# acids-ircam/RAVE

Hardware: NVIDIA H100
Metric: audio-seconds/s (v2 train step fwd+bwd, 48 kHz) (higher is better)
Workload: dtype bf16

## Files before the change

### include/rave_b200.h

```cpp
#ifndef RAVE_B200_H
#define RAVE_B200_H

#include <stddef.h>
#include <stdint.h>

#ifdef __cplusplus
extern "C" {
#endif

#define RAVE_ACT_NONE 0
#define RAVE_ACT_LEAKY 1
#define RAVE_ACT_SNAKE 2

#define RAVE_PREC_FP32 0
#define RAVE_PREC_BF16 1
#define RAVE_PREC_TF32 2

int rave_b200_version(void);
const char *rave_b200_last_error(void);
unsigned long long rave_b200_launch_count(void);

int rave_pqmf_analysis_fwd(const float *x, const float *taps, float *y, int B, int T, int Lout,
                           int ntaps, int pad_l, int flip_sign, void *stream);
int rave_pqmf_synthesis_fwd(const float *x, const float *w, float *out, int B, int L, int K,
// ... 18 lines not shown
int rave_conv1d_wgrad_f32(const float *P, const float *Q, float *dw, int B, int Ca, int Lp, int Cc,
                          int Lq, int K, int stride, int dil, int pad_l, long os_a, long os_c,
                          int act_p, int act_q, float slope, const float *alpha, void *workspace,
                          void *stream);

int rave_weight_norm_fwd(const float *v, const float *g, float *w, float *norm_out, int C0, int R,
                         void *stream);
int rave_weight_norm_bwd(const float *dw, const float *v, const float *g, const float *norm,
                         float *dv, float *dg, int C0, int R, void *stream);

int rave_act_fwd(const float *x, float *y, int B, int C, int L, int act, float slope,
                 const float *alpha, void *stream);
int rave_act_bwd(const float *dy, const float *x, float *dx, float *dalpha, int B, int C, int L,
                 int act, float slope, const float *alpha, void *stream);
int rave_am_tanh_fwd(const float *x, float *y, int B, int C, int L, void *stream);
int rave_am_tanh_bwd(const float *dy, const float *x, float *dx, int B, int C, int L, void *stream);
int rave_reparam_fwd(const float *z, const float *eps, float *zs, float *kl_sum, int B, int C, int L, void *stream);
int rave_mmd_fwd(const float *z, const float *prior, float *means, float *mmd, int B, int D, int L, void *stream);
int rave_mmd_bwd(const float *z, const float *prior, const float *g, float *dz, int B, int D, int L, void *stream);
int rave_sphere_norm_fwd(const float *z, float *out, float *norm, int B, int C, int L, void *stream);
int  rave_latent_moments(const float *z, int B, int C, int L, int D, double *state, double *work, void *stream);
long rave_latent_moments_workspace_bytes(int B, int L, int D);
int rave_sphere_norm_bwd(const float *g, const float *out, const float *norm, float *dz, int B, int C, int L,
                         void *stream);

int rave_conv1d_tc_supported(int Cin, int Cout, int K, int stride, int dil);
int rave_dilated_unit_tc_supported(int C, int L);
int rave_dilated_unit_tc_fwd(const void *xa_bf16, const void *w3t_bf16, const void *w1t_bf16, void *a1_out,
                             float *out_f32, void *out_act, int B, int C, int L, int pitch, int dil, int pad_l,
                             float slope_in, float slope_mid, int act_out, float slope_out, void *stream);
int rave_conv1d_tc_plan(int B, int Cin, int Cout, int Lout, int K);
int rave_conv1d_tc_pp_stages(int B, int Cin, int Cout, int Lout, int K, int fm, int res_bf16);
int rave_conv1d_tc_pp_fwd_stages(int B, int Cin, int Cout, int Lout, int K);
int rave_conv1d_tc_fwd(const void *xa_bf16, const void *wt_bf16, const float *bias, const float *res,
                       const void *res_bf16, const void *dact_src_bf16, const void *res_act_bf16, float res_slope,
                       float *out_f32, void *out_act_bf16,
                       int B, int Cin, int Lin, int in_pitch, int Cout, int Lout,
                       int K, int stride, int dil, int pad_l, int act, float slope, int out_rows,
                       int out_row_stride, int out_row_offset, const float *fm_d, int fm_bh, void *stream);
int rave_conv1d_tc_fwd_x3(const void *xa_bf16, const void *wt_bf16, const float *bias, const float *res,
                          const void *res_act, float res_slope, float *out_f32, void *out_act, int B, int Cin, int Lin,
                          int in_pitch, int Cout, int Lout, int K, int stride, int dil, int pad_l, int act, float slope,
                          int out_rows, int out_row_stride, int out_row_offset, int act_cs, void *stream);
int rave_conv1d_tc_wgrad_splits(int B, int Cm, int Lp, int Cn, int K);
int rave_conv1d_tc_wgrad_plan(int B, int Cm, int Lp, int Cn, int K);
int rave_time_stack_cl(const float *x, void *out_bf16, int B, int C, int T, int F, int Fp, int Cp, int kt, int pt,
                       void *stream);
int rave_time_stack_cl_bwd(const void *g_bf16, float *gx, int B, int C, int T, int F, int Fp, int Cp, int kt, int pt,
                           void *stream);
int rave_time_stack_nhwc(const float *x, void *out_bf16, int B, int C, int T, int F, long sb, long st, int Fp, int Cp, int kt,
                         int pt, void *stream);
int rave_time_stack_nhwc_bwd(const void *g_bf16, float *gx, int B, int C, int T, int F, int Fp, int Cp, int kt, int pt,
                             void *stream);
int rave_time_stack_nhwc_dil(const float *x, void *out_bf16, int B, int C, int T, int F, long sb, long st, int Fp, int Cp,
                             int kt, int pt, int dil, void *stream);
int rave_time_stack_nhwc_dil_bwd(const void *g_bf16, float *gx, int B, int C, int T, int F, int Fp, int Cp, int kt, int pt,
                                 int dil, void *stream);
int rave_l1_stats_f32(const float *t, const float *v, float *stats, long n, void *stream);
int rave_l1_grad_f32(const float *t, const float *v, const float *d, float *gt, float *gv, long n, void *stream);
int rave_leaky_fm_fwd(const float *x, float *a, float *stats, long H, float slope, void *stream);
int rave_leaky_fm_bwd(const float *a, const float *g, const float *d, float *gx, long H, float slope, void *stream);
int rave_leaky_fm_stack_fwd(const float *x, float *a, float *stats, void *xs_bf16, long Rh, int T, int F, int C, int Fp,
                            float slope, void *stream);
int rave_leaky_fm_stack_bwd(const float *a, const void *gxs_bf16, const float *ga, const float *d, float *gx, long Rh, int T,
                            int F, int C, int Fp, float slope, void *stream);
int rave_leaky_fm_stack_dil_fwd(const float *x, float *a, float *stats, void *xs_bf16, long Rh, int T, int F, int C, int Fp,
// ... 136 lines not shown
```

### rave_b200/_lib.py

```python
import ctypes
import os
from ctypes import c_float, c_int, c_long, c_longlong, c_size_t, c_ulonglong, c_void_p, c_char_p

_HERE = os.path.dirname(os.path.abspath(__file__))
LIB_PATH = os.path.join(_HERE, "csrc", "librave_b200.so")

_P, _I, _F, _L = c_void_p, c_int, c_float, c_long

SIGNATURES = {
    "rave_b200_version": (c_int, []),
    "rave_b200_last_error": (c_char_p, []),
    "rave_b200_launch_count": (c_ulonglong, []),
    "rave_pqmf_analysis_fwd": (c_int, [_P, _P, _P, _I, _I, _I, _I, _I, _I, _P]),
    "rave_pqmf_synthesis_fwd": (c_int, [_P, _P, _P, _I, _I, _I, _I, _F, _I, _P]),
    "rave_pqmf_analysis_fast": (c_int, [_P, _P, _P, _P, _I, _I, _I, _I, _I, _P]),
    "rave_pqmf_synthesis_fast": (c_int, [_P, _P, _P, _P, _I, _I, _I, _F, _I, _P]),
    "rave_conv1d_gather_f32": (c_int, [_P, _P, _P, _P, _P, _I, _I, _I, _I, _I, _I, _I, _I, _I, _L, _L,
                                       _I, _F, _P, _I, _F, _P, _P, _P]),
    "rave_conv1d_scatter_f32": (c_int, [_P, _P, _P, _P, _P, _I, _I, _I, _I, _I, _I, _I, _I, _I, _L, _L,
                                        _I, _F, _P, _I, _F, _P, _P, _P]),
    "rave_conv1d_wgrad_workspace_bytes": (c_size_t, [_I, _I, _I, _I, _I]),
    "rave_conv1d_wgrad_f32": (c_int, [_P, _P, _P, _I, _I, _I, _I, _I, _I, _I, _I, _I, _L, _L, _I, _I,
                                      _F, _P, _P, _P]),
    "rave_weight_norm_fwd": (c_int, [_P, _P, _P, _P, _I, _I, _P]),
    "rave_weight_norm_bwd": (c_int, [_P, _P, _P, _P, _P, _P, _I, _I, _P]),
    "rave_act_fwd": (c_int, [_P, _P, _I, _I, _I, _I, _F, _P, _P]),
    "rave_act_bwd": (c_int, [_P, _P, _P, _P, _I, _I, _I, _I, _F, _P, _P]),
    "rave_am_tanh_fwd": (c_int, [_P, _P, _I, _I, _I, _P]),
    "rave_am_tanh_bwd": (c_int, [_P, _P, _P, _I, _I, _I, _P]),
    "rave_reparam_fwd": (c_int, [_P, _P, _P, _P, _I, _I, _I, _P]),
    "rave_mmd_fwd": (c_int, [_P, _P, _P, _P, _I, _I, _I, _P]),
    "rave_mmd_bwd": (c_int, [_P, _P, _P, _P, _I, _I, _I, _P]),
    "rave_sphere_norm_fwd": (c_int, [_P, _P, _P, _I, _I, _I, _P]),
    "rave_sphere_norm_bwd": (c_int, [_P, _P, _P, _P, _I, _I, _I, _P]),
    "rave_latent_moments": (c_int, [_P, _I, _I, _I, _I, _P, _P, _P]),
    "rave_latent_moments_workspace_bytes": (c_long, [_I, _I, _I]),
    "rave_conv1d_tc_supported": (c_int, [_I, _I, _I, _I, _I]),
    "rave_dilated_unit_tc_supported": (c_int, [_I, _I]),
    "rave_dilated_unit_tc_fwd": (c_int, [_P, _P, _P, _P, _P, _P, _I, _I, _I, _I, _I, _I, _F, _F, _I, _F, _P]),
    "rave_conv1d_tc_plan": (c_int, [_I, _I, _I, _I, _I]),
    "rave_conv1d_tc_pp_stages": (c_int, [_I, _I, _I, _I, _I, _I, _I]),
    "rave_conv1d_tc_pp_fwd_stages": (c_int, [_I, _I, _I, _I, _I]),
    "rave_conv1d_tc_fwd": (c_int, [_P, _P, _P, _P, _P, _P, _P, _F, _P, _P, _I, _I, _I, _I, _I, _I, _I, _I, _I, _I, _I,
                                   _F, _I, _I, _I, _P, _I, _P]),
    "rave_conv1d_tc_fwd_x3": (c_int, [_P, _P, _P, _P, _P, _F, _P, _P, _I, _I, _I, _I, _I, _I, _I, _I, _I, _I, _I, _F, _I,
                                      _I, _I, _I, _P]),
    "rave_weight_prep_tc_multi_x3": (c_int, [_I, _P, _P]),
    "rave_ncl_to_cl_x3": (c_int, [_P, _P, _I, _I, _I, _P]),
    "rave_conv1d_tc_wgrad": (c_int, [_P, _P, _P, _P, _I, _I, _I, _I, _I, _I, _I, _I, _I, _I, _I, _P]),
    "rave_tapmajor_to_weight_f32": (c_int, [_P, _P, _I, _I, _I, _I, _I, _P]),
    "rave_conv1d_tc_wgrad_splits": (c_int, [_I, _I, _I, _I, _I]),
    "rave_conv1d_tc_wgrad_plan": (c_int, [_I, _I, _I, _I, _I]),
    "rave_time_stack_cl": (c_int, [_P, _P, _I, _I, _I, _I, _I, _I, _I, _I, _P]),
    "rave_time_stack_cl_bwd": (c_int, [_P, _P, _I, _I, _I, _I, _I, _I, _I, _I, _P]),
    "rave_time_stack_nhwc": (c_int, [_P, _P, _I, _I, _I, _I, ctypes.c_long, ctypes.c_long, _I, _I, _I, _I, _P]),
    "rave_time_stack_nhwc_bwd": (c_int, [_P, _P, _I, _I, _I, _I, _I, _I, _I, _I, _P]),
    "rave_time_stack_nhwc_dil": (c_int, [_P, _P, _I, _I, _I, _I, ctypes.c_long, ctypes.c_long, _I, _I, _I, _I, _I, _P]),
    "rave_time_stack_nhwc_dil_bwd": (c_int, [_P, _P, _I, _I, _I, _I, _I, _I, _I, _I, _I, _P]),
    "rave_l1_stats_f32": (c_int, [_P, _P, _P, ctypes.c_long, _P]),
    "rave_leaky_fm_fwd": (c_int, [_P, _P, _P, ctypes.c_long, ctypes.c_float, _P]),
    "rave_leaky_fm_bwd": (c_int, [_P, _P, _P, _P, ctypes.c_long, ctypes.c_float, _P]),
    "rave_leaky_fm_stack_fwd": (c_int, [_P, _P, _P, _P, ctypes.c_long, _I, _I, _I, _I, ctypes.c_float, _P]),
    "rave_leaky_fm_stack_bwd": (c_int, [_P, _P, _P, _P, _P, ctypes.c_long, _I, _I, _I, _I, ctypes.c_float, _P]),
    "rave_leaky_fm_stack_dil_fwd": (c_int, [_P, _P, _P, _P, ctypes.c_long, _I, _I, _I, _I, _I, ctypes.c_float, _P]),
    "rave_leaky_fm_stack_dil_bwd": (c_int, [_P, _P, _P, _P, _P, ctypes.c_long, _I, _I, _I, _I, _I, ctypes.c_float, _P]),
    "rave_l1_grad_f32": (c_int, [_P, _P, _P, _P, _P, ctypes.c_long, _P]),
    "rave_snake_cl_fwd": (c_int, [_P, _P, _P, ctypes.c_long, _I, _P]),
    "rave_snake_cl_bwd": (c_int, [_P, _P, _P, _P, _P, _P, ctypes.c_long, _I, _P]),
    "rave_adain_cl_stats": (c_int, [_P, _I, _I, _I, _I, _P, _P, _P, _P, _P, _P, _P, _P, _I, _P, _P, _P]),
    "rave_adain_snake_cl_fwd": (c_int, [_P, _P, _P, _P, _P, _I, _I, _I, _I, _P]),
    "rave_weight_prep_tc": (c_int, [_P, _P, _P, _P, _P, _I, _P, _P, _I, _I, _I, _I, _I, _I, _P]),
    "rave_weight_norm_bwd_tapmajor": (c_int, [_P, _P, _P, _P, _P, _P, _I, _I, _I, _I, _I, _I, _P]),
    "rave_conv1d_c1_fwd": (c_int, [_P, _P, _P, _P, _P, _I, _I, _I, _I, _I, _I, _I, _I, _I, _I, _F, _P]),
    "rave_conv1d_c1_wgrad_splits": (c_int, [_I, _I]),
    "rave_conv1d_c1_wgrad": (c_int, [_P, _P, _P, _I, _I, _I, _I, _I, _I, _I, _I, _I, _I, _P]),
# ... 127 lines not shown
```

### rave_b200/csrc/conv_tc.cu

```cuda
#include <string.h>

#include <type_traits>

#include "common.cuh"
#include "tc_common.cuh"

namespace rave {
namespace tc {

constexpr int BLOCK_M = 128;
constexpr int NUM_THREADS = 288;
constexpr int SMEM_MAX = 227 * 1024;

struct TcParams {
  int B, Cin, Lin, Cout, Lout, K, stride, dil, pad_l;
  int BL, BB;
  int n_lt, n_bg, n_nt;
  int num_kb;
  int act;
  float slope;
  const float *bias;
  const float *res;
  const __nv_bfloat16 *res_bf16;
  const __nv_bfloat16 *dact_src;
// ... 227 lines not shown

struct Ring {
  uint64_t *full, *empty;
  int stages;
  int stage;
  uint32_t phase;
  __device__ __forceinline__ void advance() {
    if (++stage == stages) { stage = 0; phase ^= 1; }
  }
};

template <int BLOCK_N, int BLOCK_K, bool X3>
__device__ __forceinline__ void produce_kblock(uint8_t *smem, Ring &r, const CUtensorMap *tmap_a,
                                               const CUtensorMap *tmap_b, const TcParams &p, const TileCoord &t,
                                               TapOrigin o, int k, int kb) {
  using L = SmemLayout<BLOCK_N, BLOCK_K, X3>;
  mbar_wait(&r.empty[r.stage], r.phase ^ 1);
  uint8_t *sa = smem + r.stage * L::STAGE_BYTES;
  uint8_t *sb = sa + L::A_BYTES;
  uint64_t *bar = &r.full[r.stage];
  if (elect_one()) {
    mbar_arrive_expect_tx(bar, L::A_BYTES + L::B_BYTES);
    tma_load_4d(sa, tmap_a, bar, kb * BLOCK_K, o.ph, t.l0 + o.j, t.b0);
    tma_load_2d(sb, tmap_b, bar, kb * BLOCK_K, k * p.Cout + t.n0);
    if (X3) {
      tma_load_4d(sa + L::A_PART, tmap_a, bar, p.Cin + kb * BLOCK_K, o.ph, t.l0 + o.j, t.b0);
      tma_load_2d(sb + L::B_PART, tmap_b, bar, kb * BLOCK_K, (p.K + k) * p.Cout + t.n0);
    }
  }
  __syncwarp();
  r.advance();
}

template <int BLOCK_N, int BLOCK_K, bool X3>
__device__ __forceinline__ void mma_kblock(float (*d)[BLOCK_N / 2], uint32_t sa, int kb) {
  using L = SmemLayout<BLOCK_N, BLOCK_K, X3>;
  constexpr int SWZ = BLOCK_K * 2;
  constexpr uint64_t A_HALF = (64 * SWZ) >> 4;
  const uint64_t adesc = make_kmajor_desc(sa, SWZ);
  const uint64_t bdesc = make_kmajor_desc(sa + L::A_BYTES, SWZ);
  wgmma_fence();
#pragma unroll
  for (int kk = 0; kk < BLOCK_K / 16; ++kk) {
#pragma unroll
    for (int h = 0; h < 2; ++h)
      Wgmma<BLOCK_N, 0, 0>::mma(d[h], adesc + h * A_HALF + 2 * kk, bdesc + 2 * kk, (kb > 0 || kk > 0) ? 1u : 0u);
  }
  if (X3) {
    const uint64_t adesc_lo = make_kmajor_desc(sa + L::A_PART, SWZ);
    const uint64_t bdesc_lo = make_kmajor_desc(sa + L::A_BYTES + L::B_PART, SWZ);
#pragma unroll
    for (int kk = 0; kk < BLOCK_K / 16; ++kk) {
#pragma unroll
      for (int h = 0; h < 2; ++h) {
        Wgmma<BLOCK_N, 0, 0>::mma(d[h], adesc_lo + h * A_HALF + 2 * kk, bdesc + 2 * kk, 1u);
        Wgmma<BLOCK_N, 0, 0>::mma(d[h], adesc + h * A_HALF + 2 * kk, bdesc_lo + 2 * kk, 1u);
      }
    }
  }
  wgmma_commit();
}

template <int BLOCK_N, int BLOCK_K, bool X3>
__device__ __forceinline__ int mma_mainloop(float (*d)[BLOCK_N / 2], uint32_t smem_base, Ring &r, int kblocks,
                                            int lane) {
  using L = SmemLayout<BLOCK_N, BLOCK_K, X3>;
  int prev = 0;
  for (int kb = 0; kb < kblocks; ++kb) {
    mbar_wait(&r.full[r.stage], r.phase);
    mma_kblock<BLOCK_N, BLOCK_K, X3>(d, smem_base + r.stage * L::STAGE_BYTES, kb);
    wgmma_wait<1>();
    if (kb > 0) {
      __syncwarp();
      if (lane == 0) mbar_arrive(&r.empty[prev]);
    }
    prev = r.stage;
    r.advance();
  }
  return prev;
}

template <int BLOCK_N>
__device__ __forceinline__ void mma_drain(float (*d)[BLOCK_N / 2], const Ring &r, int prev, int lane) {
  wgmma_wait<0>();
  wgmma_fence_regs<BLOCK_N / 2>(d[0]);
  wgmma_fence_regs<BLOCK_N / 2>(d[1]);
  __syncwarp();
  if (lane == 0) mbar_arrive(&r.empty[prev]);
}

template <int BLOCK_N, int BLOCK_K, bool X3>
__global__ void __launch_bounds__(NUM_THREADS, 1)
conv_tc_kernel(const __grid_constant__ CUtensorMap tmap_a, const __grid_constant__ CUtensorMap tmap_b,
               const __grid_constant__ CUtensorMap tmap_o, const TcParams p) {
  using L = SmemLayout<BLOCK_N, BLOCK_K, X3>;
  const int STAGES = p.stages;
  static_assert(BLOCK_N % 16 == 0 && BLOCK_N >= 16 && BLOCK_N <= 128, "invalid wgmma N");

  extern __shared__ uint8_t smem_raw[];
  uint8_t *smem = reinterpret_cast<uint8_t *>((reinterpret_cast<uintptr_t>(smem_raw) + 1023) & ~uintptr_t(1023));
  uint64_t *full_bar = reinterpret_cast<uint64_t *>(smem + p.bar_off);
  uint64_t *empty_bar = full_bar + STAGES;
  uint64_t *tfull_bar = empty_bar + STAGES;
  uint64_t *tempty_bar = tfull_bar + 2;
  uint8_t *stg = (!X3 && p.stg) ? smem + p.stg_off : nullptr;

  const int warp = threadIdx.x >> 5;
  const int lane = threadIdx.x & 31;
  const int num_tiles = p.n_lt * p.n_bg * p.n_nt;
  const int kblocks = p.K * p.num_kb;

  if (threadIdx.x == 0) {
    tma_prefetch_desc(&tmap_a);
    tma_prefetch_desc(&tmap_b);
    if (stg) tma_prefetch_desc(&tmap_o);
    for (int s = 0; s < STAGES; ++s) {
      mbar_init(&full_bar[s], 1);
      mbar_init(&empty_bar[s], 4);
    }
// ... 75 lines not shown

enum PpEpi : int { PP_FM = 1, PP_RS = 2, PP_FWD = 4, PP_BIAS = 8, PP_LEAKY = 16 };

template <int BLOCK_N, int BOXC, bool FM, bool RS>
__device__ __forceinline__ void pp_epilogue(float (*d)[BLOCK_N / 2], uint8_t *slot, const TcParams &p, int w, int lane,
                                            int b0) {
  constexpr int TILE_BYTES = BLOCK_M * BLOCK_N * 2;
  uint8_t *part = slot + TILE_BYTES;
  uint8_t *skip = slot + (FM ? 2 : 1) * TILE_BYTES;
  constexpr int SPAN = BOXC * 2, JB = BOXC / 8;
  const float d0 = FM ? __ldg(p.fm_d) : 0.f, d1 = FM ? __ldg(p.fm_d + 1) : 0.f;
  const uint32_t base = stg_offset<BOXC>(16 * w + (lane >> 2), 0) + 4 * (lane & 3);
#pragma unroll
  for (int h = 0; h < 2; ++h) {
#pragma unroll
    for (int r = 0; r < 2; ++r) {
      const int row = 64 * h + 16 * w + (lane >> 2) + 8 * r;
      const float d1r = (FM && b0 + row / p.BL < p.fm_bh) ? d1 : 0.f;
#pragma unroll
      for (int j = 0; j < BLOCK_N / 8; ++j) {
        const uint32_t off = (base ^ (uint32_t)((j % JB) << 4)) + (j / JB) * (BLOCK_M * SPAN) + (64 * h + 8 * r) * SPAN;
        float v0 = d[h][4 * j + 2 * r], v1 = d[h][4 * j + 2 * r + 1];
        const uint32_t dm = *reinterpret_cast<const uint32_t *>(slot + off);
        lrelu_mask(v0, v1, dm, p.slope);
        if (FM) fm_grad(v0, v1, dm, *reinterpret_cast<const uint32_t *>(part + off), d0, d1r);
        if (RS) add_bf16_pair(v0, v1, *reinterpret_cast<const uint32_t *>(skip + off));
        __nv_bfloat162 o = __floats2bfloat162_rn(v0, v1);
        *reinterpret_cast<uint32_t *>(slot + off) = *reinterpret_cast<uint32_t *>(&o);
      }
    }
  }
}

template <int BLOCK_N, int BOXC, bool BIAS, bool LEAKY>
__device__ __forceinline__ void pp_fwd_epilogue(float (*d)[BLOCK_N / 2], uint8_t *slot, const TcParams &p, int w,
                                                int lane, int n0) {
  constexpr int SPAN = BOXC * 2, JB = BOXC / 8;
  const uint32_t base = stg_offset<BOXC>(16 * w + (lane >> 2), 0) + 4 * (lane & 3);
  const uint32_t sslot = smem_u32(slot);
  const float2 *bias = reinterpret_cast<const float2 *>(p.bias + n0 + 2 * (lane & 3));
#pragma unroll
  for (int j = 0; j < BLOCK_N / 8; ++j) {
    const float2 bb = BIAS ? __ldg(bias + 4 * j) : make_float2(0.f, 0.f);
    const uint32_t col = (base ^ (uint32_t)((j % JB) << 4)) + (j / JB) * (BLOCK_M * SPAN);
#pragma unroll
    for (int h = 0; h < 2; ++h) {
#pragma unroll
      for (int r = 0; r < 2; ++r) {
        float v0 = d[h][4 * j + 2 * r], v1 = d[h][4 * j + 2 * r + 1];
        if (BIAS) {
          v0 += bb.x;
          v1 += bb.y;
        }
        if (LEAKY) {
          v0 = fmaxf(v0, v0 * p.slope);
          v1 = fmaxf(v1, v1 * p.slope);
        }
        __nv_bfloat162 o = __floats2bfloat162_rn(v0, v1);
        asm volatile("st.shared.b32 [%0], %1;" ::"r"(sslot + col + (64 * h + 8 * r) * SPAN),
                     "r"(*reinterpret_cast<uint32_t *>(&o))
                     : "memory");
      }
    }
  }
}

template <int BLOCK_N, int BLOCK_K, int E>
__device__ __forceinline__ void conv_tc_pp_body(const CUtensorMap *tmap_a, const CUtensorMap *tmap_b,
                                                const CUtensorMap *tmap_m, const CUtensorMap *tmap_p,
                                                const CUtensorMap *tmap_r, const CUtensorMap *tmap_o,
                                                const TcParams &p) {
  using L = SmemLayout<BLOCK_N, BLOCK_K, false>;
  constexpr int BOXC = L::OUT_BOXC;
  constexpr int BOX_BYTES = BLOCK_M * L::OUT_SPAN;
  constexpr int TILE_BYTES = BLOCK_M * BLOCK_N * 2;
  constexpr bool FWD = E & PP_FWD, FM = E & PP_FM, RS = E & PP_RS;
  const int STAGES = p.stages;
  static_assert(BLOCK_N % 16 == 0 && BLOCK_N >= 16 && BLOCK_N <= 128, "invalid wgmma N");
  static_assert(!FWD || !(FM || RS), "the forward epilogue has no gradient operands");

  extern __shared__ uint8_t smem_raw[];
  uint8_t *smem = reinterpret_cast<uint8_t *>((reinterpret_cast<uintptr_t>(smem_raw) + 1023) & ~uintptr_t(1023));
  uint64_t *full_bar = reinterpret_cast<uint64_t *>(smem + p.bar_off);
  uint64_t *empty_bar = full_bar + STAGES;
  uint64_t *ofull_bar = empty_bar + STAGES;
  uint64_t *oempty_bar = ofull_bar + 2;
  uint64_t *order_bar = oempty_bar + 2;

  const int wg = threadIdx.x >> 7;
  const int warp = threadIdx.x >> 5;
  const int lane = threadIdx.x & 31;
  const int num_tiles = p.n_lt * p.n_bg * p.n_nt;
// ... 88 lines not shown
      fence_proxy_async();
      named_bar_sync(1 + c, 128);
      if (issuer) {
#pragma unroll
        for (int cb = 0; cb < BLOCK_N / BOXC; ++cb)
          tma_store_3d(tmap_o, slot + cb * BOX_BYTES, t.n0 + cb * BOXC, t.l0, t.b0);
        bulk_commit();
        bulk_wait_read<0>();
        mbar_arrive(&oempty_bar[c]);
      }
    }
    if (issuer) bulk_wait_all();
  }
}

template <int BLOCK_N, int BLOCK_K, bool FM, bool RS>
__global__ void __launch_bounds__(PP_THREADS, 1)
conv_tc_pp_kernel(const __grid_constant__ CUtensorMap tmap_a, const __grid_constant__ CUtensorMap tmap_b,
                  const __grid_constant__ CUtensorMap tmap_m, const __grid_constant__ CUtensorMap tmap_p,
                  const __grid_constant__ CUtensorMap tmap_r, const __grid_constant__ CUtensorMap tmap_o,
                  const TcParams p) {
  conv_tc_pp_body<BLOCK_N, BLOCK_K, (FM ? PP_FM : 0) | (RS ? PP_RS : 0)>(&tmap_a, &tmap_b, &tmap_m, &tmap_p, &tmap_r,
                                                                         &tmap_o, p);
}

template <int BLOCK_N, int BLOCK_K, bool BIAS, bool LEAKY>
__global__ void __launch_bounds__(PP_THREADS, 1)
conv_tc_pp_fwd_kernel(const __grid_constant__ CUtensorMap tmap_a, const __grid_constant__ CUtensorMap tmap_b,
                      const __grid_constant__ CUtensorMap tmap_o, const TcParams p) {
  conv_tc_pp_body<BLOCK_N, BLOCK_K, PP_FWD | (BIAS ? PP_BIAS : 0) | (LEAKY ? PP_LEAKY : 0)>(
      &tmap_a, &tmap_b, nullptr, nullptr, nullptr, &tmap_o, p);
}

static CUtensorMapSwizzle swizzle_enum(int bytes) {
  return bytes == 128 ? CU_TENSOR_MAP_SWIZZLE_128B : bytes == 64 ? CU_TENSOR_MAP_SWIZZLE_64B
                                                                 : CU_TENSOR_MAP_SWIZZLE_32B;
}

static int pick_block_k(int Cin) {
  if (Cin % 64 == 0) return 64;
  if (Cin % 32 == 0) return 32;
  if (Cin % 16 == 0) return 16;
  return 0;
}

static int pick_block_n(int Cout, long m_tiles) {
  const int cands[] = {128, 96, 64, 48, 32, 16};
  constexpr int NC = sizeof(cands) / sizeof(cands[0]);
  int best = 0;
  for (int c : cands) {
    if (Cout % c) continue;
    if (!best) best = c;
    if (m_tiles * (Cout / c) >= 132) return c;
  }
  for (int i = NC - 1; i >= 0; --i)
    if (Cout % cands[i] == 0 && cands[i] >= 32) return cands[i];
  return best;
}

struct TcGeometry {
  int BK, BL, BB, n_lt, n_bg, BN, n_nt, num_kb;
};
static TcGeometry tc_geometry(int B, int Cin, int Cout, int Lout) {
  TcGeometry g;
  g.BK = pick_block_k(Cin);
  g.BL = 128;
// ... 34 lines not shown

template <int BN>
static int encode_rows_map(CUtensorMap *m, const __nv_bfloat16 *base, const TcParams &p, int box_b) {
  using L = SmemLayout<BN, 64, false>;
  const cuuint64_t dims[3] = {(cuuint64_t)p.Cout, (cuuint64_t)p.Lout, (cuuint64_t)p.B};
  const cuuint64_t strides[2] = {(cuuint64_t)p.Cout * 2 * p.out_row_stride, (cuuint64_t)p.Cout * 2 * p.out_rows};
  const cuuint32_t box[3] = {(cuuint32_t)L::OUT_BOXC, (cuuint32_t)p.BL, (cuuint32_t)box_b};
  const CUresult r = encode_bf16_map(m, 3, base + (size_t)p.out_row_offset * p.Cout, dims, strides, box,
                                     swizzle_enum(L::OUT_SPAN), CU_TENSOR_MAP_L2_PROMOTION_NONE);
  if (r != CUDA_SUCCESS) {
    set_error("conv1d_tc: bf16 row tensor map encode failed (%d)", (int)r);
    return 1;
  }
  return 0;
}

template <int BN, int BK, bool FWD>
constexpr bool pp_built = FWD || !(BN == 96 && BK == 64);

template <int BN, int BK, bool FWD>
constexpr int pp_stages(int nops) {
  using L = SmemLayout<BN, BK, false>;
  if (!pp_built<BN, BK, FWD>) return 0;
  const int s = (SMEM_MAX - L::FIXED - 2 * nops * BLOCK_M * BN * 2) / L::STAGE_BYTES;
  return s < 2 ? 0 : s > 8 ? 8 : s;
}

template <int BN, int BK>
static int pp_fwd_stages(int kblocks) {
  const int s = pp_stages<BN, BK, true>(1);
  TcParams q;
  plan_smem<BN, BK, false>(kblocks, q);
  return s >= q.stages && (BN == 128 || kblocks <= 24) ? s : 0;
}

template <int BN, int BK, bool FWD>
static int launch_pp(const CUtensorMap &ta, const CUtensorMap &tb, TcParams p, int stages, cudaStream_t stream) {
  using L = SmemLayout<BN, BK, false>;
  p.stages = stages;
  p.ops_bytes = (1 + (p.fm_d ? 1 : 0) + (p.res_bf16 ? 1 : 0)) * BLOCK_M * BN * 2;
  p.ops_off = p.stages * L::STAGE_BYTES;
  p.bar_off = p.ops_off + 2 * p.ops_bytes;
  const int grid = persistent_grid(p.n_lt * p.n_bg * p.n_nt), smem = p.bar_off + L::FIXED;
  const std::true_type y;
  const std::false_type n;
  CUtensorMap tm, tp, tr, to;
  if (encode_rows_map<BN>(&to, p.out_act, p, p.BB)) return 1;
  if constexpr (FWD) {
    const auto go = [&](auto bias, auto leaky) {
      return launch_tc<conv_tc_pp_fwd_kernel<BN, BK, decltype(bias)::value, decltype(leaky)::value>>(
          "conv1d_tc", grid, PP_THREADS, smem, stream, ta, tb, to, p);
    };
    const bool leaky = p.act == RAVE_ACT_LEAKY;
    return p.bias ? (leaky ? go(y, y) : go(y, n)) : (leaky ? go(n, y) : go(n, n));
  } else {
    memset(&tp, 0, sizeof(tp));
    memset(&tr, 0, sizeof(tr));
    if (encode_rows_map<BN>(&tm, p.dact_src, p, p.BB)) return 1;
    if (p.fm_d && encode_rows_map<BN>(&tp, p.fm_bh > 0 ? p.dact_src : p.dact_src - p.fm_half, p, 1)) return 1;
    if (p.res_bf16 && encode_rows_map<BN>(&tr, p.res_bf16, p, p.BB)) return 1;
    const auto go = [&](auto fm, auto rs) {
      return launch_tc<conv_tc_pp_kernel<BN, BK, decltype(fm)::value, decltype(rs)::value>>(
          "conv1d_tc", grid, PP_THREADS, smem, stream, ta, tb, tm, tp, tr, to, p);
    };
    return p.fm_d ? (p.res_bf16 ? go(y, y) : go(y, n)) : (p.res_bf16 ? go(n, y) : go(n, n));
  }
// ... 32 lines not shown
}

extern "C" int rave_conv1d_tc_plan(int B, int Cin, int Cout, int Lout, int K) {
  using namespace rave::tc;
  const TcGeometry g = tc_geometry(B, Cin, Cout, Lout);
  if (!g.BK || !g.BN) return 0;
  TcParams q;
  visit_tile(g.BK, g.BN, [&](auto bk, auto bn) {
    plan_smem<decltype(bn)::value, decltype(bk)::value, false>(K * g.num_kb, q);
    return 0;
  });
  return g.BN | (g.BK << 12) | (q.nacc - 1) << 24 | q.stg << 25 | q.stages << 26;
}

extern "C" int rave_conv1d_tc_pp_stages(int B, int Cin, int Cout, int Lout, int K, int fm, int res_bf16) {
  using namespace rave::tc;
  const TcGeometry g = tc_geometry(B, Cin, Cout, Lout);
  if (!g.BK || !g.BN) return 0;
  const int nops = 1 + (fm ? 1 : 0) + (res_bf16 ? 1 : 0);
  return visit_tile(g.BK, g.BN, [&](auto bk, auto bn) {
    return pp_stages<decltype(bn)::value, decltype(bk)::value, false>(nops);
  });
}

extern "C" int rave_conv1d_tc_pp_fwd_stages(int B, int Cin, int Cout, int Lout, int K) {
  using namespace rave::tc;
  const TcGeometry g = tc_geometry(B, Cin, Cout, Lout);
  if (!g.BK || !g.BN) return 0;
  return visit_tile(g.BK, g.BN, [&](auto bk, auto bn) {
    return pp_fwd_stages<decltype(bn)::value, decltype(bk)::value>(K * g.num_kb);
  });
}

static int conv1d_tc_fwd_impl(const void *xa, const void *wt, const float *bias, const float *res,
                              const void *res_bf16, const void *dact_src, const void *res_act, float res_slope,
                              float *out_f32, void *out_act,
                              int B, int Cin, int Lin, int in_pitch, int Cout, int Lout,
                              int K, int stride, int dil, int pad_l, int act, float slope, int out_rows,
                              int out_row_stride, int out_row_offset, const float *fm_d, int fm_bh,
                              void *stream, int x3, int act_cs = 0) {
  using namespace rave;
  using namespace rave::tc;
  RAVE_CHECK_ARG(!x3 || (!res_bf16 && !dact_src && !fm_d),
                 "conv1d_tc(x3): the split-operand mode has no gradient epilogues (forward path only)");
  RAVE_CHECK_ARG(xa && wt && (out_f32 || out_act), "conv1d_tc: null pointer");
  RAVE_CHECK_ARG(rave_conv1d_tc_supported(Cin, Cout, K, stride, dil), "conv1d_tc: unsupported shape Cin=%d Cout=%d",
                 Cin, Cout);
  if (in_pitch <= 0) in_pitch = Lin;
  RAVE_CHECK_ARG(in_pitch >= ceil_div(Lin, stride) * stride,
                 "conv1d_tc: input pitch %d < Lin %d rounded up to the stride %d (slack rows must be zero)", in_pitch,
                 Lin, stride);
  RAVE_CHECK_ARG(act == RAVE_ACT_NONE || act == RAVE_ACT_LEAKY, "conv1d_tc: epilogue activation %d unsupported", act);
  RAVE_CHECK_ARG(act != RAVE_ACT_LEAKY || (slope >= 0.f && slope <= 1.f), "conv1d_tc: LeakyReLU slope %g outside [0, 1]",
                 (double)slope);
  RAVE_CHECK_ARG(!res_act || (res_slope > 0.f && res_slope <= 1.f), "conv1d_tc: res_slope %g outside (0, 1]",
                 (double)res_slope);
  RAVE_CHECK_ARG(((uintptr_t)bias & 15) == 0, "conv1d_tc: bias must be 16-byte aligned");
  RAVE_CHECK_ARG(((uintptr_t)xa & 15) == 0 && ((uintptr_t)wt & 15) == 0, "conv1d_tc: operands must be 16B aligned");
  RAVE_CHECK_ARG((((uintptr_t)out_f32 | (uintptr_t)out_act | (uintptr_t)res | (uintptr_t)res_bf16 | (uintptr_t)dact_src |
                   (uintptr_t)res_act) & 31) == 0,
                 "conv1d_tc: epilogue tensors must be 32-byte aligned (256-bit row segments)");
  RAVE_CHECK_ARG(get_encode_fn(), "conv1d_tc: cuTensorMapEncodeTiled not available");

  const TcGeometry g = tc_geometry(B, Cin, Cout, Lout);
  RAVE_CHECK_ARG(g.BN > 0, "conv1d_tc: no BLOCK_N for Cout=%d", Cout);
  const int BK = g.BK, BN = g.BN;
  const CUtensorMapL2promotion promo = BK == 64 ? CU_TENSOR_MAP_L2_PROMOTION_L2_256B : CU_TENSOR_MAP_L2_PROMOTION_NONE;
  TcParams p;
  p.B = B; p.Cin = Cin; p.Lin = Lin; p.Cout = Cout; p.Lout = Lout; p.K = K; p.stride = stride; p.dil = dil;
  p.pad_l = pad_l; p.act = act; p.slope = slope; p.bias = bias; p.res = res; p.out_f32 = out_f32;
  p.res_bf16 = (const __nv_bfloat16 *)res_bf16; p.dact_src = (const __nv_bfloat16 *)dact_src;
  p.res_act = (const __nv_bfloat16 *)res_act;
  p.res_inv_slope = (res_act && res_slope > 0.f) ? 1.f / res_slope : 1.f;
  p.out_act = (__nv_bfloat16 *)out_act;
  p.out_rows = out_rows > 0 ? out_rows : Lout;
  p.out_row_stride = out_row_stride > 0 ? out_row_stride : 1;
  p.out_row_offset = out_row_offset;
  RAVE_CHECK_ARG(!fm_d || (dact_src && slope > 0.f && ((fm_bh > 0 && 2 * fm_bh == B) || (fm_bh < 0 && -fm_bh == B))),
                 "conv1d_tc: the fused feature-matching gradient needs dact_src and a [real; fake] batch (B=%d, fm_bh=%d)",
                 B, fm_bh);
  p.fm_d = fm_d;
  p.fm_bh = fm_bh > 0 ? fm_bh : 0;
  p.fm_half = (long)(fm_bh > 0 ? fm_bh : -fm_bh) * p.out_rows * Cout;
  p.act_ld = x3 ? 2 * Cout : Cout;
  p.act_cs = act_cs > 0 ? act_cs : Cout;
  RAVE_CHECK_ARG(!x3 || (Cout % p.act_cs == 0 && p.act_cs % 16 == 0),
                 "conv1d_tc(x3): %d channels per position do not tile the %d-column rows in 16-column chunks", p.act_cs,
                 Cout);
  RAVE_CHECK_ARG(!x3 || !res_act || p.act_cs == Cout, "conv1d_tc(x3): res_act needs one position per row");
  p.BL = g.BL; p.BB = g.BB; p.n_lt = g.n_lt; p.n_bg = g.n_bg; p.n_nt = g.n_nt; p.num_kb = g.num_kb;

  CUtensorMap ta, tb;
  {
    const cuuint64_t ca = (cuuint64_t)Cin * (x3 ? 2 : 1);
    const cuuint64_t dims[4] = {ca, (cuuint64_t)stride, (cuuint64_t)ceil_div(Lin, stride), (cuuint64_t)B};
    const cuuint64_t strides[3] = {ca * 2, ca * 2 * stride, ca * 2 * in_pitch};
    const cuuint32_t box[4] = {(cuuint32_t)BK, 1, (cuuint32_t)p.BL, (cuuint32_t)p.BB};
    const CUresult r = encode_bf16_map(&ta, 4, xa, dims, strides, box, swizzle_enum(BK * 2), promo);
    RAVE_CHECK_ARG(r == CUDA_SUCCESS, "conv1d_tc: tensor map A encode failed (%d)", (int)r);
  }
  {
    const cuuint64_t dims[2] = {(cuuint64_t)Cin, (cuuint64_t)K * Cout * (x3 ? 2 : 1)};
    const cuuint64_t strides[1] = {(cuuint64_t)Cin * 2};
    const cuuint32_t box[2] = {(cuuint32_t)BK, (cuuint32_t)BN};
    const CUresult r = encode_bf16_map(&tb, 2, wt, dims, strides, box, swizzle_enum(BK * 2), promo);
    RAVE_CHECK_ARG(r == CUDA_SUCCESS, "conv1d_tc: tensor map B encode failed (%d)", (int)r);
  }
  cudaStream_t s = (cudaStream_t)stream;
  if (x3) return conv_tc_dispatch_x3(BK, BN, ta, tb, p, s);
  const bool bf16_only = out_act && !res && !res_act && !out_f32;
  const bool pp_dgrad = bf16_only && dact_src && !bias && act == RAVE_ACT_NONE;
  const bool pp_fwd = bf16_only && !dact_src && !res_bf16 && !fm_d;
  const int nops = 1 + (fm_d ? 1 : 0) + (res_bf16 ? 1 : 0);
  return visit_tile(BK, BN, [&](auto bk, auto bn) {
    constexpr int BK_ = decltype(bk)::value, BN_ = decltype(bn)::value;
    if constexpr (pp_built<BN_, BK_, false>) {
      const int stages = pp_dgrad ? pp_stages<BN_, BK_, false>(nops) : 0;
      if (stages) return launch_pp<BN_, BK_, false>(ta, tb, p, stages, s);
    }
    if constexpr (pp_built<BN_, BK_, true>) {
      const int stages = pp_fwd ? pp_fwd_stages<BN_, BK_>(K * g.num_kb) : 0;
      if (stages) return launch_pp<BN_, BK_, true>(ta, tb, p, stages, s);
    }
    return launch<BN_, BK_, false>(ta, tb, p, s);
  });
}

extern "C" int rave_conv1d_tc_fwd(const void *xa, const void *wt, const float *bias, const float *res,
                                  const void *res_bf16, const void *dact_src, const void *res_act, float res_slope,
                                  float *out_f32, void *out_act,
                                  int B, int Cin, int Lin, int in_pitch, int Cout, int Lout,
                                  int K, int stride, int dil, int pad_l, int act, float slope, int out_rows,
                                  int out_row_stride, int out_row_offset, const float *fm_d, int fm_bh,
                                  void *stream) {
  return conv1d_tc_fwd_impl(xa, wt, bias, res, res_bf16, dact_src, res_act, res_slope, out_f32, out_act, B, Cin, Lin,
                            in_pitch, Cout, Lout, K, stride, dil, pad_l, act, slope, out_rows, out_row_stride,
                            out_row_offset, fm_d, fm_bh, stream, 0);
}

extern "C" int rave_conv1d_tc_fwd_x3(const void *xa, const void *wt, const float *bias, const float *res,
                                     const void *res_act, float res_slope, float *out_f32, void *out_act,
                                     int B, int Cin, int Lin, int in_pitch, int Cout, int Lout,
                                     int K, int stride, int dil, int pad_l, int act, float slope, int out_rows,
                                     int out_row_stride, int out_row_offset, int act_cs, void *stream) {
  return conv1d_tc_fwd_impl(xa, wt, bias, res, nullptr, nullptr, res_act, res_slope, out_f32, out_act, B, Cin, Lin,
// ... 320 lines not shown
```

### rave_b200/csrc/wgmma_sm90.cuh

```cuda
#pragma once
#include <stdint.h>

namespace rave {
namespace tc {

template <int N, int TA, int TB>
struct Wgmma;

template <int TA, int TB>
struct Wgmma<16, TA, TB> {
  __device__ static __forceinline__ void mma(float *d, uint64_t a, uint64_t b, uint32_t scale_d) {
    asm volatile(
        "{\n\t.reg .pred p;\n\tsetp.ne.b32 p, %10, 0;\n\t"
        "wgmma.mma_async.sync.aligned.m64n16k16.f32.bf16.bf16 {%0, %1, %2, %3, %4, %5, %6, %7}, %8, %9, p, 1, 1, %11, %12;\n\t}"
        : "+f"(d[0]), "+f"(d[1]), "+f"(d[2]), "+f"(d[3]), "+f"(d[4]), "+f"(d[5]), "+f"(d[6]), "+f"(d[7])
        : "l"(a), "l"(b), "r"(scale_d), "n"(TA), "n"(TB));
  }
};

template <int TA, int TB>
struct Wgmma<32, TA, TB> {
  __device__ static __forceinline__ void mma(float *d, uint64_t a, uint64_t b, uint32_t scale_d) {
    asm volatile(
        "{\n\t.reg .pred p;\n\tsetp.ne.b32 p, %18, 0;\n\t"
// ... 17 lines not shown
template <int TA, int TB>
struct Wgmma<64, TA, TB> {
  __device__ static __forceinline__ void mma(float *d, uint64_t a, uint64_t b, uint32_t scale_d) {
    asm volatile(
        "{\n\t.reg .pred p;\n\tsetp.ne.b32 p, %34, 0;\n\t"
        "wgmma.mma_async.sync.aligned.m64n64k16.f32.bf16.bf16 {%0, %1, %2, %3, %4, %5, %6, %7, %8, %9, %10, %11, %12, %13, %14, %15, %16, %17, %18, %19, %20, %21, %22, %23, %24, %25, %26, %27, %28, %29, %30, %31}, %32, %33, p, 1, 1, %35, %36;\n\t}"
        : "+f"(d[0]), "+f"(d[1]), "+f"(d[2]), "+f"(d[3]), "+f"(d[4]), "+f"(d[5]), "+f"(d[6]), "+f"(d[7]), "+f"(d[8]), "+f"(d[9]), "+f"(d[10]), "+f"(d[11]), "+f"(d[12]), "+f"(d[13]), "+f"(d[14]), "+f"(d[15]), "+f"(d[16]), "+f"(d[17]), "+f"(d[18]), "+f"(d[19]), "+f"(d[20]), "+f"(d[21]), "+f"(d[22]), "+f"(d[23]), "+f"(d[24]), "+f"(d[25]), "+f"(d[26]), "+f"(d[27]), "+f"(d[28]), "+f"(d[29]), "+f"(d[30]), "+f"(d[31])
        : "l"(a), "l"(b), "r"(scale_d), "n"(TA), "n"(TB));
  }
};

template <int TA, int TB>
struct Wgmma<96, TA, TB> {
  __device__ static __forceinline__ void mma(float *d, uint64_t a, uint64_t b, uint32_t scale_d) {
    asm volatile(
        "{\n\t.reg .pred p;\n\tsetp.ne.b32 p, %50, 0;\n\t"
        "wgmma.mma_async.sync.aligned.m64n96k16.f32.bf16.bf16 {%0, %1, %2, %3, %4, %5, %6, %7, %8, %9, %10, %11, %12, %13, %14, %15, %16, %17, %18, %19, %20, %21, %22, %23, %24, %25, %26, %27, %28, %29, %30, %31, %32, %33, %34, %35, %36, %37, %38, %39, %40, %41, %42, %43, %44, %45, %46, %47}, %48, %49, p, 1, 1, %51, %52;\n\t}"
        : "+f"(d[0]), "+f"(d[1]), "+f"(d[2]), "+f"(d[3]), "+f"(d[4]), "+f"(d[5]), "+f"(d[6]), "+f"(d[7]), "+f"(d[8]), "+f"(d[9]), "+f"(d[10]), "+f"(d[11]), "+f"(d[12]), "+f"(d[13]), "+f"(d[14]), "+f"(d[15]), "+f"(d[16]), "+f"(d[17]), "+f"(d[18]), "+f"(d[19]), "+f"(d[20]), "+f"(d[21]), "+f"(d[22]), "+f"(d[23]), "+f"(d[24]), "+f"(d[25]), "+f"(d[26]), "+f"(d[27]), "+f"(d[28]), "+f"(d[29]), "+f"(d[30]), "+f"(d[31]), "+f"(d[32]), "+f"(d[33]), "+f"(d[34]), "+f"(d[35]), "+f"(d[36]), "+f"(d[37]), "+f"(d[38]), "+f"(d[39]), "+f"(d[40]), "+f"(d[41]), "+f"(d[42]), "+f"(d[43]), "+f"(d[44]), "+f"(d[45]), "+f"(d[46]), "+f"(d[47])
        : "l"(a), "l"(b), "r"(scale_d), "n"(TA), "n"(TB));
  }
};

template <int TA, int TB>
struct Wgmma<128, TA, TB> {
  __device__ static __forceinline__ void mma(float *d, uint64_t a, uint64_t b, uint32_t scale_d) {
    asm volatile(
        "{\n\t.reg .pred p;\n\tsetp.ne.b32 p, %66, 0;\n\t"
        "wgmma.mma_async.sync.aligned.m64n128k16.f32.bf16.bf16 {%0, %1, %2, %3, %4, %5, %6, %7, %8, %9, %10, %11, %12, %13, %14, %15, %16, %17, %18, %19, %20, %21, %22, %23, %24, %25, %26, %27, %28, %29, %30, %31, %32, %33, %34, %35, %36, %37, %38, %39, %40, %41, %42, %43, %44, %45, %46, %47, %48, %49, %50, %51, %52, %53, %54, %55, %56, %57, %58, %59, %60, %61, %62, %63}, %64, %65, p, 1, 1, %67, %68;\n\t}"
        : "+f"(d[0]), "+f"(d[1]), "+f"(d[2]), "+f"(d[3]), "+f"(d[4]), "+f"(d[5]), "+f"(d[6]), "+f"(d[7]), "+f"(d[8]), "+f"(d[9]), "+f"(d[10]), "+f"(d[11]), "+f"(d[12]), "+f"(d[13]), "+f"(d[14]), "+f"(d[15]), "+f"(d[16]), "+f"(d[17]), "+f"(d[18]), "+f"(d[19]), "+f"(d[20]), "+f"(d[21]), "+f"(d[22]), "+f"(d[23]), "+f"(d[24]), "+f"(d[25]), "+f"(d[26]), "+f"(d[27]), "+f"(d[28]), "+f"(d[29]), "+f"(d[30]), "+f"(d[31]), "+f"(d[32]), "+f"(d[33]), "+f"(d[34]), "+f"(d[35]), "+f"(d[36]), "+f"(d[37]), "+f"(d[38]), "+f"(d[39]), "+f"(d[40]), "+f"(d[41]), "+f"(d[42]), "+f"(d[43]), "+f"(d[44]), "+f"(d[45]), "+f"(d[46]), "+f"(d[47]), "+f"(d[48]), "+f"(d[49]), "+f"(d[50]), "+f"(d[51]), "+f"(d[52]), "+f"(d[53]), "+f"(d[54]), "+f"(d[55]), "+f"(d[56]), "+f"(d[57]), "+f"(d[58]), "+f"(d[59]), "+f"(d[60]), "+f"(d[61]), "+f"(d[62]), "+f"(d[63])
        : "l"(a), "l"(b), "r"(scale_d), "n"(TA), "n"(TB));
  }
};

}
}
```

Baseline: 2373.

## Add wide N=192 warp-specialized conv kernel with one M-half per consumer warpgroup

Adds a persistent TMA+WGMMA forward conv kernel using 192-wide N tiles, where two consumer warpgroups each own one 64-row M half instead of one warpgroup issuing both halves. It is selected for bf16-only forward convs when Cout is a multiple of 192 and there are enough k-blocks. The goal is more B-operand reuse per tile and fewer tiles and epilogue stores. In exchange it uses more accumulator registers per thread and leaves fewer ring stages in shared memory.

```diff
diff --git a/include/rave_b200.h b/include/rave_b200.h
--- a/include/rave_b200.h
+++ b/include/rave_b200.h
@@ -74,6 +74,7 @@
 int rave_conv1d_tc_plan(int B, int Cin, int Cout, int Lout, int K);
 int rave_conv1d_tc_pp_stages(int B, int Cin, int Cout, int Lout, int K, int fm, int res_bf16);
 int rave_conv1d_tc_pp_fwd_stages(int B, int Cin, int Cout, int Lout, int K);
+int rave_conv1d_tc_wide_stages(int B, int Cin, int Cout, int Lout, int K);
 int rave_conv1d_tc_fwd(const void *xa_bf16, const void *wt_bf16, const float *bias, const float *res,
                        const void *res_bf16, const void *dact_src_bf16, const void *res_act_bf16, float res_slope,
                        float *out_f32, void *out_act_bf16,
diff --git a/rave_b200/_lib.py b/rave_b200/_lib.py
--- a/rave_b200/_lib.py
+++ b/rave_b200/_lib.py
@@ -41,6 +41,7 @@
     "rave_conv1d_tc_plan": (c_int, [_I, _I, _I, _I, _I]),
     "rave_conv1d_tc_pp_stages": (c_int, [_I, _I, _I, _I, _I, _I, _I]),
     "rave_conv1d_tc_pp_fwd_stages": (c_int, [_I, _I, _I, _I, _I]),
+    "rave_conv1d_tc_wide_stages": (c_int, [_I, _I, _I, _I, _I]),
     "rave_conv1d_tc_fwd": (c_int, [_P, _P, _P, _P, _P, _P, _P, _F, _P, _P, _I, _I, _I, _I, _I, _I, _I, _I, _I, _I, _I,
                                    _F, _I, _I, _I, _P, _I, _P]),
     "rave_conv1d_tc_fwd_x3": (c_int, [_P, _P, _P, _P, _P, _F, _P, _P, _I, _I, _I, _I, _I, _I, _I, _I, _I, _I, _I, _F, _I,
diff --git a/rave_b200/csrc/conv_tc.cu b/rave_b200/csrc/conv_tc.cu
--- a/rave_b200/csrc/conv_tc.cu
+++ b/rave_b200/csrc/conv_tc.cu
@@ -283,8 +283,8 @@
   r.advance();
 }
 
-template <int BLOCK_N, int BLOCK_K, bool X3>
-__device__ __forceinline__ void mma_kblock(float (*d)[BLOCK_N / 2], uint32_t sa, int kb) {
+template <int BLOCK_N, int BLOCK_K, bool X3, int NH = 2>
+__device__ __forceinline__ void mma_kblock(float (*d)[BLOCK_N / 2], uint32_t sa, int kb, int h0 = 0) {
   using L = SmemLayout<BLOCK_N, BLOCK_K, X3>;
   constexpr int SWZ = BLOCK_K * 2;
   constexpr uint64_t A_HALF = (64 * SWZ) >> 4;
@@ -294,8 +294,8 @@
 #pragma unroll
   for (int kk = 0; kk < BLOCK_K / 16; ++kk) {
 #pragma unroll
-    for (int h = 0; h < 2; ++h)
-      Wgmma<BLOCK_N, 0, 0>::mma(d[h], adesc + h * A_HALF + 2 * kk, bdesc + 2 * kk, (kb > 0 || kk > 0) ? 1u : 0u);
+    for (int h = 0; h < NH; ++h)
+      Wgmma<BLOCK_N, 0, 0>::mma(d[h], adesc + (h0 + h) * A_HALF + 2 * kk, bdesc + 2 * kk, (kb > 0 || kk > 0) ? 1u : 0u);
   }
   if (X3) {
     const uint64_t adesc_lo = make_kmajor_desc(sa + L::A_PART, SWZ);
@@ -312,14 +312,14 @@
   wgmma_commit();
 }
 
-template <int BLOCK_N, int BLOCK_K, bool X3>
+template <int BLOCK_N, int BLOCK_K, bool X3, int NH = 2>
 __device__ __forceinline__ int mma_mainloop(float (*d)[BLOCK_N / 2], uint32_t smem_base, Ring &r, int kblocks,
-                                            int lane) {
+                                            int lane, int h0 = 0) {
   using L = SmemLayout<BLOCK_N, BLOCK_K, X3>;
   int prev = 0;
   for (int kb = 0; kb < kblocks; ++kb) {
     mbar_wait(&r.full[r.stage], r.phase);
-    mma_kblock<BLOCK_N, BLOCK_K, X3>(d, smem_base + r.stage * L::STAGE_BYTES, kb);
+    mma_kblock<BLOCK_N, BLOCK_K, X3, NH>(d, smem_base + r.stage * L::STAGE_BYTES, kb, h0);
     wgmma_wait<1>();
     if (kb > 0) {
       __syncwarp();
@@ -331,11 +331,11 @@
   return prev;
 }
 
-template <int BLOCK_N>
+template <int BLOCK_N, int NH = 2>
 __device__ __forceinline__ void mma_drain(float (*d)[BLOCK_N / 2], const Ring &r, int prev, int lane) {
   wgmma_wait<0>();
-  wgmma_fence_regs<BLOCK_N / 2>(d[0]);
-  wgmma_fence_regs<BLOCK_N / 2>(d[1]);
+#pragma unroll
+  for (int h = 0; h < NH; ++h) wgmma_fence_regs<BLOCK_N / 2>(d[h]);
   __syncwarp();
   if (lane == 0) mbar_arrive(&r.empty[prev]);
 }
@@ -477,9 +477,9 @@
   }
 }
 
-template <int BLOCK_N, int BOXC, bool BIAS, bool LEAKY>
+template <int BLOCK_N, int BOXC, bool BIAS, bool LEAKY, int NH = 2>
 __device__ __forceinline__ void pp_fwd_epilogue(float (*d)[BLOCK_N / 2], uint8_t *slot, const TcParams &p, int w,
-                                                int lane, int n0) {
+                                                int lane, int n0, int h0 = 0) {
   constexpr int SPAN = BOXC * 2, JB = BOXC / 8;
   const uint32_t base = stg_offset<BOXC>(16 * w + (lane >> 2), 0) + 4 * (lane & 3);
   const uint32_t sslot = smem_u32(slot);
@@ -489,7 +489,7 @@
     const float2 bb = BIAS ? __ldg(bias + 4 * j) : make_float2(0.f, 0.f);
     const uint32_t col = (base ^ (uint32_t)((j % JB) << 4)) + (j / JB) * (BLOCK_M * SPAN);
 #pragma unroll
-    for (int h = 0; h < 2; ++h) {
+    for (int h = 0; h < NH; ++h) {
 #pragma unroll
       for (int r = 0; r < 2; ++r) {
         float v0 = d[h][4 * j + 2 * r], v1 = d[h][4 * j + 2 * r + 1];
@@ -502,7 +502,7 @@
           v1 = fmaxf(v1, v1 * p.slope);
         }
         __nv_bfloat162 o = __floats2bfloat162_rn(v0, v1);
-        asm volatile("st.shared.b32 [%0], %1;" ::"r"(sslot + col + (64 * h + 8 * r) * SPAN),
+        asm volatile("st.shared.b32 [%0], %1;" ::"r"(sslot + col + (64 * (h0 + h) + 8 * r) * SPAN),
                      "r"(*reinterpret_cast<uint32_t *>(&o))
                      : "memory");
       }
@@ -657,6 +657,89 @@
       &tmap_a, &tmap_b, nullptr, nullptr, nullptr, &tmap_o, p);
 }
 
+constexpr int WIDE_N = 192;
+
+template <int BLOCK_K, bool BIAS, bool LEAKY>
+__global__ void __launch_bounds__(PP_THREADS, 1)
+conv_tc_wide_kernel(const __grid_constant__ CUtensorMap tmap_a, const __grid_constant__ CUtensorMap tmap_b,
+                    const __grid_constant__ CUtensorMap tmap_o, const TcParams p) {
+  constexpr int BLOCK_N = WIDE_N;
+  using L = SmemLayout<BLOCK_N, BLOCK_K, false>;
+  constexpr int BOXC = L::OUT_BOXC;
+  constexpr int BOX_BYTES = BLOCK_M * L::OUT_SPAN;
+  const int STAGES = p.stages;
+
+  extern __shared__ uint8_t smem_raw[];
+  uint8_t *smem = reinterpret_cast<uint8_t *>((reinterpret_cast<uintptr_t>(smem_raw) + 1023) & ~uintptr_t(1023));
+  uint64_t *full_bar = reinterpret_cast<uint64_t *>(smem + p.bar_off);
+  uint64_t *empty_bar = full_bar + STAGES;
+  uint64_t *oempty_bar = empty_bar + STAGES;
+
+  const int wg = threadIdx.x >> 7;
+  const int warp = threadIdx.x >> 5;
+  const int lane = threadIdx.x & 31;
+  const int num_tiles = p.n_lt * p.n_bg * p.n_nt;
+  const int kblocks = p.K * p.num_kb;
+
+  if (threadIdx.x == 0) {
+    tma_prefetch_desc(&tmap_a);
+    tma_prefetch_desc(&tmap_b);
+    tma_prefetch_desc(&tmap_o);
+    for (int s = 0; s < STAGES; ++s) {
+      mbar_init(&full_bar[s], 1);
+      mbar_init(&empty_bar[s], 8);
+    }
+    mbar_init(oempty_bar, 1);
+    fence_barrier_init();
+  }
+  __syncthreads();
+  griddep_launch_dependents();
+  griddep_wait();
+
+  Ring ring{full_bar, empty_bar, STAGES, 0, 0};
+  if (wg == 0) {
+    warpgroup_reg_dealloc<56>();
+    if (warp != 0) return;
+    for (int tile = blockIdx.x; tile < num_tiles; tile += gridDim.x) {
+      const TileCoord t = tile_coord<BLOCK_N>(tile, p);
+      for (int k = 0; k < p.K; ++k) {
+        const TapOrigin o = tap_origin(k, p.dil, p.pad_l, p.stride);
+        for (int kb = 0; kb < p.num_kb; ++kb)
+          produce_kblock<BLOCK_N, BLOCK_K, false>(smem, ring, &tmap_a, &tmap_b, p, t, o, k, kb);
+      }
+    }
+  } else {
+    warpgroup_reg_alloc<224>();
+    const int h = wg - 1;
+    const int w = warp & 3;
+    const bool issuer = threadIdx.x == 128;
+    const uint32_t smem_base = smem_u32(smem);
+    uint8_t *slot = smem + p.ops_off;
+    float d[1][BLOCK_N / 2];
+    int u = 0;
+    for (int tile = blockIdx.x; tile < num_tiles; tile += gridDim.x, ++u) {
+      const int prev = mma_mainloop<BLOCK_N, BLOCK_K, false, 1>(d, smem_base, ring, kblocks, lane, h);
+      mma_drain<BLOCK_N, 1>(d, ring, prev, lane);
+      const TileCoord t = tile_coord<BLOCK_N>(tile, p);
+      if (issuer && u > 0) {
+        bulk_wait_read<0>();
+        mbar_arrive(oempty_bar);
+      }
+      mbar_wait(oempty_bar, (u & 1) ^ 1);
+      pp_fwd_epilogue<BLOCK_N, BOXC, BIAS, LEAKY, 1>(d, slot, p, w, lane, t.n0, h);
+      fence_proxy_async();
+      named_bar_sync(1, 256);
+      if (issuer) {
+#pragma unroll
+        for (int cb = 0; cb < BLOCK_N / BOXC; ++cb)
+          tma_store_3d(&tmap_o, slot + cb * BOX_BYTES, t.n0 + cb * BOXC, t.l0, t.b0);
+        bulk_commit();
+      }
+    }
+    if (issuer) bulk_wait_all();
+  }
+}
+
 static CUtensorMapSwizzle swizzle_enum(int bytes) {
   return bytes == 128 ? CU_TENSOR_MAP_SWIZZLE_128B : bytes == 64 ? CU_TENSOR_MAP_SWIZZLE_64B
                                                                  : CU_TENSOR_MAP_SWIZZLE_32B;
@@ -757,6 +840,40 @@
   TcParams q;
   plan_smem<BN, BK, false>(kblocks, q);
   return s >= q.stages && (BN == 128 || kblocks <= 24) ? s : 0;
+}
+
+static int wide_block_k(int Cin) { return pick_block_k(Cin); }
+template <int BK>
+constexpr int wide_ring_stages() {
+  using L = SmemLayout<WIDE_N, BK, false>;
+  const int s = (SMEM_MAX - L::FIXED - L::STG_BYTES) / L::STAGE_BYTES;
+  return s > 8 ? 8 : s;
+}
+constexpr int WIDE_MIN_KBLOCKS = 12;
+static int wide_stages(int Cin, int Cout, int K) {
+  const int BK = wide_block_k(Cin);
+  if (BK < 32 || Cout % WIDE_N || K * ceil_div(Cin, BK) < WIDE_MIN_KBLOCKS) return 0;
+  return BK == 64 ? wide_ring_stages<64>() : wide_ring_stages<32>();
+}
+
+template <int BK>
+static int launch_wide(const CUtensorMap &ta, const CUtensorMap &tb, TcParams p, int stages, cudaStream_t stream) {
+  using L = SmemLayout<WIDE_N, BK, false>;
+  p.stages = stages;
+  p.ops_bytes = L::STG_BYTES;
+  p.ops_off = p.stages * L::STAGE_BYTES;
+  p.bar_off = p.ops_off + p.ops_bytes;
+  const int grid = persistent_grid(p.n_lt * p.n_bg * p.n_nt), smem = p.bar_off + L::FIXED;
+  CUtensorMap to;
+  if (encode_rows_map<WIDE_N>(&to, p.out_act, p, p.BB)) return 1;
+  const auto go = [&](auto bias, auto leaky) {
+    return launch_tc<conv_tc_wide_kernel<BK, decltype(bias)::value, decltype(leaky)::value>>(
+        "conv1d_tc", grid, PP_THREADS, smem, stream, ta, tb, to, p);
+  };
+  const std::true_type y;
+  const std::false_type n;
+  const bool leaky = p.act == RAVE_ACT_LEAKY;
+  return p.bias ? (leaky ? go(y, y) : go(y, n)) : (leaky ? go(n, y) : go(n, n));
 }
 
 template <int BN, int BK, bool FWD>
@@ -855,6 +972,13 @@
   });
 }
 
+extern "C" int rave_conv1d_tc_wide_stages(int B, int Cin, int Cout, int Lout, int K) {
+  using namespace rave::tc;
+  const TcGeometry g = tc_geometry(B, Cin, Cout, Lout);
+  if (!g.BK || !g.BN) return 0;
+  return wide_stages(Cin, Cout, K);
+}
+
 static int conv1d_tc_fwd_impl(const void *xa, const void *wt, const float *bias, const float *res,
                               const void *res_bf16, const void *dact_src, const void *res_act, float res_slope,
                               float *out_f32, void *out_act,
@@ -887,7 +1011,11 @@
 
   const TcGeometry g = tc_geometry(B, Cin, Cout, Lout);
   RAVE_CHECK_ARG(g.BN > 0, "conv1d_tc: no BLOCK_N for Cout=%d", Cout);
-  const int BK = g.BK, BN = g.BN;
+  const bool bf16_only = out_act && !res && !res_act && !out_f32;
+  const bool pp_dgrad = bf16_only && dact_src && !bias && act == RAVE_ACT_NONE;
+  const bool pp_fwd = bf16_only && !dact_src && !res_bf16 && !fm_d;
+  const int wide = !x3 && pp_fwd ? wide_stages(Cin, Cout, K) : 0;
+  const int BK = wide ? wide_block_k(Cin) : g.BK, BN = wide ? WIDE_N : g.BN;
   const CUtensorMapL2promotion promo = BK == 64 ? CU_TENSOR_MAP_L2_PROMOTION_L2_256B : CU_TENSOR_MAP_L2_PROMOTION_NONE;
   TcParams p;
   p.B = B; p.Cin = Cin; p.Lin = Lin; p.Cout = Cout; p.Lout = Lout; p.K = K; p.stride = stride; p.dil = dil;
@@ -911,7 +1039,9 @@
                  "conv1d_tc(x3): %d channels per position do not tile the %d-column rows in 16-column chunks", p.act_cs,
                  Cout);
   RAVE_CHECK_ARG(!x3 || !res_act || p.act_cs == Cout, "conv1d_tc(x3): res_act needs one position per row");
-  p.BL = g.BL; p.BB = g.BB; p.n_lt = g.n_lt; p.n_bg = g.n_bg; p.n_nt = g.n_nt; p.num_kb = g.num_kb;
+  p.BL = g.BL; p.BB = g.BB; p.n_lt = g.n_lt; p.n_bg = g.n_bg;
+  p.n_nt = Cout / BN;
+  p.num_kb = ceil_div(Cin, BK);
 
   CUtensorMap ta, tb;
   {
@@ -931,9 +1061,7 @@
   }
   cudaStream_t s = (cudaStream_t)stream;
   if (x3) return conv_tc_dispatch_x3(BK, BN, ta, tb, p, s);
-  const bool bf16_only = out_act && !res && !res_act && !out_f32;
-  const bool pp_dgrad = bf16_only && dact_src && !bias && act == RAVE_ACT_NONE;
-  const bool pp_fwd = bf16_only && !dact_src && !res_bf16 && !fm_d;
+  if (wide) return BK == 64 ? launch_wide<64>(ta, tb, p, wide, s) : launch_wide<32>(ta, tb, p, wide, s);
   const int nops = 1 + (fm_d ? 1 : 0) + (res_bf16 ? 1 : 0);
   return visit_tile(BK, BN, [&](auto bk, auto bn) {
     constexpr int BK_ = decltype(bk)::value, BN_ = decltype(bn)::value;
diff --git a/rave_b200/csrc/wgmma_sm90.cuh b/rave_b200/csrc/wgmma_sm90.cuh
--- a/rave_b200/csrc/wgmma_sm90.cuh
+++ b/rave_b200/csrc/wgmma_sm90.cuh
@@ -73,5 +73,16 @@
   }
 };
 
+template <int TA, int TB>
+struct Wgmma<192, TA, TB> {
+  __device__ static __forceinline__ void mma(float *d, uint64_t a, uint64_t b, uint32_t scale_d) {
+    asm volatile(
+        "{\n\t.reg .pred p;\n\tsetp.ne.b32 p, %98, 0;\n\t"
+        "wgmma.mma_async.sync.aligned.m64n192k16.f32.bf16.bf16 {%0, %1, %2, %3, %4, %5, %6, %7, %8, %9, %10, %11, %12, %13, %14, %15, %16, %17, %18, %19, %20, %21, %22, %23, %24, %25, %26, %27, %28, %29, %30, %31, %32, %33, %34, %35, %36, %37, %38, %39, %40, %41, %42, %43, %44, %45, %46, %47, %48, %49, %50, %51, %52, %53, %54, %55, %56, %57, %58, %59, %60, %61, %62, %63, %64, %65, %66, %67, %68, %69, %70, %71, %72, %73, %74, %75, %76, %77, %78, %79, %80, %81, %82, %83, %84, %85, %86, %87, %88, %89, %90, %91, %92, %93, %94, %95}, %96, %97, p, 1, 1, %99, %100;\n\t}"
+        : "+f"(d[0]), "+f"(d[1]), "+f"(d[2]), "+f"(d[3]), "+f"(d[4]), "+f"(d[5]), "+f"(d[6]), "+f"(d[7]), "+f"(d[8]), "+f"(d[9]), "+f"(d[10]), "+f"(d[11]), "+f"(d[12]), "+f"(d[13]), "+f"(d[14]), "+f"(d[15]), "+f"(d[16]), "+f"(d[17]), "+f"(d[18]), "+f"(d[19]), "+f"(d[20]), "+f"(d[21]), "+f"(d[22]), "+f"(d[23]), "+f"(d[24]), "+f"(d[25]), "+f"(d[26]), "+f"(d[27]), "+f"(d[28]), "+f"(d[29]), "+f"(d[30]), "+f"(d[31]), "+f"(d[32]), "+f"(d[33]), "+f"(d[34]), "+f"(d[35]), "+f"(d[36]), "+f"(d[37]), "+f"(d[38]), "+f"(d[39]), "+f"(d[40]), "+f"(d[41]), "+f"(d[42]), "+f"(d[43]), "+f"(d[44]), "+f"(d[45]), "+f"(d[46]), "+f"(d[47]), "+f"(d[48]), "+f"(d[49]), "+f"(d[50]), "+f"(d[51]), "+f"(d[52]), "+f"(d[53]), "+f"(d[54]), "+f"(d[55]), "+f"(d[56]), "+f"(d[57]), "+f"(d[58]), "+f"(d[59]), "+f"(d[60]), "+f"(d[61]), "+f"(d[62]), "+f"(d[63]), "+f"(d[64]), "+f"(d[65]), "+f"(d[66]), "+f"(d[67]), "+f"(d[68]), "+f"(d[69]), "+f"(d[70]), "+f"(d[71]), "+f"(d[72]), "+f"(d[73]), "+f"(d[74]), "+f"(d[75]), "+f"(d[76]), "+f"(d[77]), "+f"(d[78]), "+f"(d[79]), "+f"(d[80]), "+f"(d[81]), "+f"(d[82]), "+f"(d[83]), "+f"(d[84]), "+f"(d[85]), "+f"(d[86]), "+f"(d[87]), "+f"(d[88]), "+f"(d[89]), "+f"(d[90]), "+f"(d[91]), "+f"(d[92]), "+f"(d[93]), "+f"(d[94]), "+f"(d[95])
+        : "l"(a), "l"(b), "r"(scale_d), "n"(TA), "n"(TB));
+  }
+};
+
 }
 }
```

New measurement: 2484 (median of 6 runs). 1.05x the previous value.
